# quenotl/PARESIS

Measured on AMD Instinct MI355X. Metric: Mpixels/s, 4096^2 Fresnel+refraction step, higher is better.
Workload: dtype f32; 1 GPU; 4096x4096 fp32 study grid, 1 membrane position per GPU per step, 4 propagation distances z={1.6,3.6,5.2,7.2} m: 4 x (Fresnel propagation + refraction) from the 2-material membrane thickness maps (transmission evaluated inside the step); 52 keV, dSM/dMO/dOD=140/1.6/3.6 m; fresnel_engine=lds, streams=1, parallelism=single GPU

## Files before the change

### paresis_amd/csrc/fresnel_p2.hip

```cpp
#include "fresnel_p2.hpp"

#include <atomic>

#include "fresnel_p2_dev.hpp"

using namespace psx;
using namespace psx::lines;
using namespace psx::p2dev;

namespace {

constexpr int TE = 512;
constexpr int TLD = 256;
constexpr int TT = TE + TLD;
constexpr int TOT2 = 16384;
constexpr int LXM = psx::p2::LXMAX;

template <int R1_, bool DUAL_>
struct G2 {
    static constexpr int R1 = R1_, M = 256 * R1, LINES = TOT2 / M, LH = DUAL_ ? LINES / 2 : LINES;
    static constexpr int MP = M + M / 32 + LXM;
    static constexpr int NBA = 32 / R1;
    static constexpr int SPL = M / 16;
    static constexpr int LB = R1 == 32 ? 5 : (R1 == 16 ? 4 : (R1 == 8 ? 3 : 2));
    static constexpr int LDP = LB | 1, LDB = 17;
    static constexpr int TPL = TLD / LINES, NCH = TPL >= 2 * LXM ? TPL / LXM : 1, CL = LXM / NCH;
    static constexpr int O_TP = LINES * MP, O_TB = O_TP + 256 * LDP, O_SA = O_TB + 16 * LDB, O_C = O_SA + LH * LXM,
                         O_UQ = O_C + NCH * LINES * LXM, O_HT = O_UQ + 2;
    static constexpr size_t lds_bytes(int ntap) { return sizeof(float2) * (size_t)(O_HT + ntap * LXM); }
    static constexpr int max_taps = (160 * 1024 / (int)sizeof(float2) - O_HT) / LXM < MAX_LINE ? (160 * 1024 / (int)sizeof(float2) - O_HT) / LXM : MAX_LINE;
    static_assert(LINES >= 2 && NBA >= 1 && max_taps >= 16, "LDS budget");
};

#define PSX_STAMP(k) PSX_STAMP_IF(k, tid == 0)

template <int R1, bool CONTIG, bool DUAL, bool QUEUE>
__global__ __launch_bounds__(TT) void k_fresnel_p2(LineArgs a) {
    using GE = G2<R1, DUAL>;
    constexpr int M = GE::M, LINES = GE::LINES, LH = GE::LH, MP = GE::MP, NBA = GE::NBA, SPL = GE::SPL, LDP = GE::LDP, LDB = GE::LDB;
    constexpr int NCH = GE::NCH, CL = GE::CL, TPL = GE::TPL;
    constexpr int LPG = LH;
    constexpr int LL = LH;
    static_assert(!DUAL || CONTIG, "DUAL is pass 1");
    extern __shared__ __attribute__((aligned(16))) float2 lds[];
    v2f *const Lb = reinterpret_cast<v2f *>(lds);
    v2f *const tP = Lb + GE::O_TP, *const tB = Lb + GE::O_TB;
    v2f *const SA = Lb + GE::O_SA;
    v2f *const CF = Lb + GE::O_C;
    v2f *const HT = Lb + GE::O_HT;
    int *const uq = reinterpret_cast<int *>(Lb + GE::O_UQ);
    const int tid = threadIdx.x;
    const int N = a.N, mg = a.margin;
    const int Lx = a.L - M;
    const bool upper_half = ((a.P - 1) >> 8) >= R1 / 2;

    const int ngroups = (a.nlines + LPG - 1) / LPG;
    const int nwork = a.dist_inner ? ngroups : ngroups * a.n_dist;
    const int xcd = blockIdx.x & 7, slot = blockIdx.x >> 3, nslot = gridDim.x >> 3;
    const int cq = nwork >> 3, cr = nwork & 7;
    const int cstart = xcd * cq + (xcd < cr ? xcd : cr), clen = cq + (xcd < cr ? 1 : 0);
    const int nunits = slot < clen ? (clen - slot + nslot - 1) / nslot : 0;
    const int nsub = DUAL ? (a.n_dist + 1) / 2 : a.n_dist;
    const int nj = a.dist_inner ? nunits * nsub : nunits;
    constexpr bool DYN = QUEUE;
    const int nsubr = a.dist_inner ? nsub : 1;
    auto item = [&](int j, int &d, int &g) __attribute__((always_inline)) {
        if (a.dist_inner) {
            const int u = j / nsub;
            d = j - u * nsub;
            g = cstart + (DYN ? uq[u & 3] : slot + u * nslot);
        } else {
            const int wk = cstart + (DYN ? uq[j & 3] : slot + j * nslot);
            d = wk / ngroups;
            g = wk - d * ngroups;
        }
    };
    auto valid = [&](int j) __attribute__((always_inline)) { return DYN ? uq[(j / nsubr) & 3] >= 0 : j < nj; };
    auto qcount = [&](int v) __attribute__((always_inline)) { return &a.queue[16 * (xcd + 8 * v)]; };
    auto share = [&](int v) __attribute__((always_inline)) { return v < clen ? (clen - v + nslot - 1) / nslot : 0; };
    bool dry = false, own_dry = false;
    const int myshare = share(slot);
    auto steal = [&]() __attribute__((always_inline)) {
        const int ln = tid & 63;
        for (int attempt = 0; attempt < 2; ++attempt) {
            const int v = ln;
            bool avail = false;
            if (v < nslot && v != slot)
                avail = __hip_atomic_load(qcount(v), __ATOMIC_RELAXED, __HIP_MEMORY_SCOPE_AGENT) < (unsigned)share(v);
            const unsigned long long m = __ballot(avail);
            if (m == 0ull) {
                dry = true;
                return -1;
            }
            const unsigned long long hi = m >> ((slot + 1) & 63);
            const int pick = hi ? (slot + 1 + __builtin_ctzll(hi)) : __builtin_ctzll(m);
            unsigned k = 0u;
            if (ln == 0) k = atomicAdd(qcount(pick), 1u);
            k = __builtin_amdgcn_readfirstlane(k);
            if (k < (unsigned)share(pick)) return pick + (int)k * nslot;
        }
        return -1;
    };

    unsigned first2 = 0u;
    if (DYN && tid == TE) first2 = atomicAdd(qcount(slot), 2u);
    for (int idx = tid; idx < 256 * GE::LB; idx += TT) {
        const float2 wv = a.twA[idx];
        tP[(idx / GE::LB) * LDP + idx % GE::LB] = (v2f){wv.x, wv.y};
    }
    for (int idx = tid; idx < 256; idx += TT) {
        const float2 w = a.twB[idx];
        tB[(idx >> 4) * LDB + (idx & 15)] = (v2f){w.x, w.y};
    }
    {
        const int ntap = DUAL ? 2 * nsub : a.n_dist;
        for (int idx = tid; idx < ntap * LXM; idx += TT) {
            const float2 h = a.H[idx / LXM][M + idx % LXM];
            HT[idx] = (v2f){h.x, h.y};
        }
    }
    if constexpr (DYN) {
        if (tid == TE) {
            uq[0] = first2 < (unsigned)myshare ? slot + (int)first2 * nslot : -1;
            uq[1] = first2 + 1u < (unsigned)myshare ? slot + (int)(first2 + 1u) * nslot : -1;
        }
        lds_barrier();
    }

    if (tid >= TE) {
        const int lt = tid - TE;
        constexpr int STEP = TLD / LL, NLD = M / (2 * STEP), PSTEP = STEP + STEP / 32;
        static_assert(TLD % LL == 0 && NLD * STEP == M / 2, "sample ownership covers M / 2 samples of every line");
        constexpr bool AFFL = (STEP % 32 == 0);
        const int line = CONTIG ? lt / STEP : lt % LL, i0 = CONTIG ? lt % STEP : lt / LL;
        const int nmir = LL * 2 * mg;
        const int lm = lt % LL;
        int im = -1, jm = 0;
        if (lt < nmir) {
            const int r = lt / LL;
            im = r < mg ? r + 1 : N - 1 - 2 * mg + r;
            jm = r < mg ? N + 2 * mg - 1 - im : 2 * N - 3 - im;
        }
        float2 *base = lds + line * MP;
        const int ja = i0 + N + 2 * mg - 1, jb = i0 - 1;
        const int oa = phys(ja), ob = phys(jb);
        float2 *sa_line = lds + GE::O_SA + line * LXM;

        constexpr int CH = LL / 2 > 0 ? LL / 2 : 1, STEPV = TLD / CH, NLV = M / (2 * STEPV), PSTEPV = STEPV + STEPV / 32;
        static_assert(CONTIG || (LL % 2 == 0 && IB % 2 == 0 && STEPV % 32 == 0 && NLV * STEPV == M / 2), "16-byte loads of the blocked intermediate");
        const int c2 = lt % CH, i0v = lt / CH;
        float2 *base_v = lds + 2 * c2 * MP;
        const int jav = i0v + N + 2 * mg - 1, jbv = i0v - 1;
        const int oav = phys(jav), obv = phys(jbv);
        float2 *sa_v = lds + GE::O_SA + 2 * c2 * LXM;
        const int voff_v = ((((2 * c2) / IB) * N + i0v) * IB + (2 * c2) % IB) * (int)sizeof(float2);

        float2 xs[CONTIG ? NLD : 1], xm = make_float2(0.f, 0.f);
        float4 xv[CONTIG ? 1 : NLV];
        auto fetch = [&](int j) __attribute__((always_inline)) {
            int d, g;
            item(j, d, g);
            if (a.dist_inner && d != 0) return;
            const float2 *src = a.src[d];
            const int l0 = g * LPG;
            if constexpr (!CONTIG) {
                constexpr int LLB = LL > IB ? LL / IB : 1;
                const int nblk = min(LLB, (a.nlines - l0 + IB - 1) / IB);
                const __amdgpu_buffer_rsrc_t rs = __builtin_amdgcn_make_buffer_rsrc(
                    const_cast<float2 *>(src) + ((int64_t)(l0 / IB) * N) * IB + l0 % IB, 0,
                    nblk * N * IB * (int)sizeof(float2) - (l0 % IB) * (int)sizeof(float2), 0x00020000);
#pragma unroll
                for (int k = 0; k < NLV; ++k) {
                    const v4u r = __builtin_amdgcn_raw_buffer_load_b128(rs, voff_v + k * (STEPV * IB * (int)sizeof(float2)), 0, 0);
                    xv[k] = __builtin_bit_cast(float4, r);
                }
                const int64_t pixm = ((int64_t)((l0 + lm) / IB) * N + im) * IB + (l0 + lm) % IB;
                xm = src[(im >= 0 && l0 + lm < a.nlines) ? pixm : (int64_t)0];
                return;
            } else {
                const __amdgpu_buffer_rsrc_t rs = __builtin_amdgcn_make_buffer_rsrc(
                    const_cast<float2 *>(src) + (int64_t)l0 * a.in_sl, 0, min(LL, a.nlines - l0) * (int)a.in_sl * (int)sizeof(float2), 0x00020000);
                const int voff = (line * (int)a.in_sl + i0) * (int)sizeof(float2);
#pragma unroll
                for (int k = 0; k < NLD; ++k) {
                    const v2u r = __builtin_amdgcn_raw_buffer_load_b64(rs, voff + k * (STEP * (int)sizeof(float2)), 0, 0);
                    xs[k] = __builtin_bit_cast(float2, r);
                }
                const int64_t pixm = (int64_t)im + (int64_t)(l0 + lm) * a.in_sl;
                xm = src[(im >= 0 && l0 + lm < a.nlines) ? pixm : (int64_t)0];
                return;
            }
        };
        auto spread = [&](int j) __attribute__((always_inline)) {
            int d, g;
            item(j, d, g);
            const int l0 = g * LPG;
            const bool line_ok = l0 + line < a.nlines;
            for (int jz = a.L + lt; jz < M; jz += TLD) {
                const int pz = phys(jz);
#pragma unroll
                for (int ln = 0; ln < LL; ++ln) lds[ln * MP + pz] = make_float2(0.f, 0.f);
            }
            if constexpr (!CONTIG) {
                const bool ok0 = l0 + 2 * c2 < a.nlines, ok1 = l0 + 2 * c2 + 1 < a.nlines;
#pragma unroll
                for (int k = 0; k < NLV; ++k) {
                    if (i0v + STEPV * k < N) {
                        const float2 x0 = ok0 ? make_float2(xv[k].x, xv[k].y) : make_float2(0.f, 0.f);
                        const float2 x1 = ok1 ? make_float2(xv[k].z, xv[k].w) : make_float2(0.f, 0.f);
                        base_v[oav + k * PSTEPV] = x0;
                        base_v[MP + oav + k * PSTEPV] = x1;
                        if (k > 0 || jbv >= 0) {
                            base_v[obv + k * PSTEPV] = x0;
                            base_v[MP + obv + k * PSTEPV] = x1;
                        }
                        if (STEPV * k <= LXM) {
                            const int js = jbv + STEPV * k;
                            if ((unsigned)js < (unsigned)LXM) {
                                sa_v[js] = x0;
                                sa_v[LXM + js] = x1;
                            }
                        }
                    }
                }
            }
#pragma unroll
            for (int k = 0; k < (CONTIG ? NLD : 0); ++k) {
                if (i0 + STEP * k < N) {
                    const float2 x = line_ok ? xs[k] : make_float2(0.f, 0.f);
                    if (AFFL) {
                        base[oa + k * PSTEP] = x;
                        if (k > 0 || jb >= 0) base[ob + k * PSTEP] = x;
                    } else {
                        base[phys(ja + STEP * k)] = x;
                        if (k > 0 || jb >= 0) base[phys(jb + STEP * k)] = x;
                    }
                    if (STEP * k <= LXM) {
                        const int js = jb + STEP * k;
                        if ((unsigned)js < (unsigned)LXM) sa_line[js] = x;
                    }
                }
            }
            if (im >= 0) lds[lm * MP + phys(jm)] = l0 + lm < a.nlines ? xm : make_float2(0.f, 0.f);
            for (int t = lt + TLD; t < nmir; t += TLD) {
                const int ln = t % LL, r = t / LL;
                const int i2 = r < mg ? r + 1 : N - 1 - 2 * mg + r, j2 = r < mg ? N + 2 * mg - 1 - i2 : 2 * N - 3 - i2;
                float2 x2 = make_float2(0.f, 0.f);
                if (l0 + ln < a.nlines)
                    x2 = a.src[d][a.in_blocked ? ((int64_t)((l0 + ln) / IB) * N + i2) * IB + (l0 + ln) % IB
                                            : (int64_t)i2 * a.in_si + (int64_t)(l0 + ln) * a.in_sl];
                lds[ln * MP + phys(j2)] = x2;
            }
        };
        auto fixup = [&](int j) __attribute__((always_inline)) {
            if (Lx <= 0) return;
            int d, g;
            item(j, d, g);
            int lo = lt;
            asm volatile("" : "+v"(lo));
            const int lb = lo / TPL, r = lo % TPL;
            const int lbi = DUAL ? lb % LH : lb;
            const int dd = DUAL ? 2 * d + lb / LH : d;
            const v2f *ht = HT + dd * LXM;
            const v2f *sa = SA + lbi * LXM;
            const v2f *sb = Lb + lbi * MP + M + M / 32;
            const int c = NCH > 1 ? r / LXM : 0;
            for (int mp = NCH > 1 ? r % LXM : r; mp < LXM; mp += (NCH > 1 ? LXM : TPL)) {
                v2f acc = (v2f){0.f, 0.f};
#pragma unroll
                for (int tt = 0; tt < CL; ++tt) {
                    const int t = c * CL + tt;
                    const int jx = mp >= t ? mp - t : 0;
                    const v2f dl = lds_read(sb + jx) - lds_read(sa + jx);
                    const v2f term = pk_cmul(dl, lds_read(ht + t));
                    acc += mp >= t ? term : (v2f){0.f, 0.f};
                }
                CF[(c * LINES + lb) * LXM + mp] = acc;
            }
        };

        if (valid(0)) {
            fetch(0);
            spread(0);
        }
        lds_barrier();
        int ucur = 0, usub = 0;
        auto ring_ok = [&](int u) __attribute__((always_inline)) { return uq[u & 3] >= 0; };
        for (int j = 0; DYN ? ring_ok(ucur) : j < nj; ++j) {
            const bool last_sub = usub + 1 == nsubr;
            const bool more = DYN ? ring_ok(last_sub ? ucur + 1 : ucur) : j + 1 < nj;
            lds_barrier();
            if (a.stamps && lt == 0 && j == a.stamp_j) a.stamps[(size_t)blockIdx.x * 32 + 16] = wall_clock64();
            const bool qround = DYN && lt < 64 && usub == 0;
            const bool claiming = qround && ring_ok(ucur + 1);
            unsigned mine = 0xffffffffu;
            if (claiming && !own_dry && lt == 0) mine = atomicAdd(qcount(slot), 1u);
            if (more) fetch(j + 1);
            if (a.stamps && lt == 0 && j == a.stamp_j) a.stamps[(size_t)blockIdx.x * 32 + 17] = wall_clock64();
            fixup(j);
            lds_barrier();
            lds_barrier();
            if (a.stamps && lt == 0 && j == a.stamp_j) a.stamps[(size_t)blockIdx.x * 32 + 18] = wall_clock64();
            __builtin_amdgcn_s_setprio(3);
            if (more) spread(j + 1);
            __builtin_amdgcn_s_setprio(0);
            if (qround) {
                int unit = -1;
                if (claiming) {
                    const unsigned k = __builtin_amdgcn_readfirstlane(mine);
                    if (k < (unsigned)myshare) unit = slot + (int)k * nslot;
                    else own_dry = true;
                    if (unit < 0 && !dry) unit = steal();
                }
                if (lt == 0) uq[(ucur + 2) & 3] = unit;
            }
            if (last_sub) {
                usub = 0;
                ++ucur;
            } else {
                ++usub;
            }
            if (a.stamps && lt == 0 && j == a.stamp_j) a.stamps[(size_t)blockIdx.x * 32 + 19] = wall_clock64();
            lds_barrier();
            if (a.stamps && lt == 0 && j == a.stamp_j) a.stamps[(size_t)blockIdx.x * 32 + 20] = wall_clock64();
        }
        if (DYN && lt < 64) {
            unsigned prev = 0u;
            if (lt == 0) {
                __threadfence();
                prev = atomicAdd(&a.queue[16 * 256], 1u);
            }
            prev = __builtin_amdgcn_readfirstlane(prev);
            if (prev == gridDim.x - 1) {
                for (int wq = lt; wq < (int)gridDim.x; wq += 64) atomicExch(&a.queue[16 * wq], 0u);
                if (lt == 0) atomicExch(&a.queue[16 * 256], 0u);
            }
        }
        return;
    }

    const int w = tid >> 6, ln = tid & 63;
    const int n3 = ln & 15, blk = ((ln >> 4) & 1) * 2 + (ln >> 5);
    const int slabw = spectrum::slab_of_lane(ln);
    const v2f *rowB = tB + n3 * LDB;
    constexpr int RPL = R1 / 4;
    const int G0 = DUAL ? 4 * w + blk : 2 * (w / RPL) * R1 + 4 * (w % RPL) + blk, G1 = G0 + (DUAL ? 32 : R1);
    const int S0 = DUAL ? 64 * w + slabw : 2 * (w / RPL) * SPL + 64 * (w % RPL) + slabw, S1 = S0 + (DUAL ? LH * SPL : SPL);
    auto block_ptr = [&](int G) __attribute__((always_inline)) { return Lb + (G / R1) * MP + (G % R1) * BSTR + n3; };
    auto slab_ptr = [&](int S) __attribute__((always_inline)) {
        const int sl = S % SPL;
        return Lb + (S / SPL) * MP + 16 * sl + (sl >> 1);
    };
    const bool fwdA_on = !(DUAL && R1 == 32) || tid < TE / 2;
    const int sg = __builtin_amdgcn_readfirstlane(w % RPL);
    const int hlane = spectrum::unit_of_lane<8>(sg, 0, ln);
    static_assert(spectrum::unit_of_lane<8>(0, 1, 0) == 64, "stride of a lane's loads");
    constexpr int NBAF = DUAL ? (R1 == 32 ? 1 : NBA / 2) : NBA;
    if (a.stamps && tid == 0) a.stamps[(size_t)blockIdx.x * 32 + 0] = wall_clock64();
    lds_barrier();
    if (a.stamps && tid == 0) a.stamps[(size_t)blockIdx.x * 32 + 1] = wall_clock64();
    int eu = 0, es = 0;
    for (int j = 0; DYN ? uq[eu & 3] >= 0 : j < nj; ++j) {
        int d, g;
        item(j, d, g);
        const int l0 = g * LPG;
        if (++es == nsubr) {
            es = 0;
            ++eu;
        }
        PSX_STAMP(2);

        if (fwdA_on) {
            v2f v[NBAF][R1], pw[5];
#pragma unroll
            for (int i = 0; i < NBAF; ++i) {
                const int b = tid + TE * i, n = b & 255;
                const v2f *p = Lb + (b >> 8) * MP + n + (n >> 5);
#pragma unroll
                for (int q = 0; q < R1; ++q) v[i][q] = p[q * BSTR];
            }
#pragma unroll
            for (int i = 0; i < NBAF; ++i) {
                const int b = tid + TE * i;
                v2f *p = Lb + (b >> 8) * MP + (b & 255) + ((b & 255) >> 5);
                DftPk<R1, false>::run(v[i]);
                __builtin_amdgcn_sched_barrier(0);
                if (i == 0) tw_powers<R1>(pw, tP + (tid & 255) * LDP);
                twiddle_A2<R1, false>(v[i], pw);
#pragma unroll
                for (int q = 0; q < R1; ++q) p[q * BSTR] = v[i][q];
            }
        }
        float4 hh[8], hh1[DUAL ? 8 : 1];
        {
            const float4 *h4 = reinterpret_cast<const float4 *>(a.H[DUAL ? 2 * d : d]) + hlane;
#pragma unroll
            for (int q = 0; q < 8; ++q) hh[q] = h4[64 * q];
        }
        PSX_STAMP(3);
        lds_barrier();
        PSX_STAMP(4);

        {
            v2f wt[16];
#pragma unroll
            for (int q = 1; q < 16; ++q) wt[q] = lds_read(rowB + q);
            wt[0] = (v2f){1.f, 0.f};
            v2f *p0 = block_ptr(G0), *p1 = block_ptr(G1);
            v2f v0[16], v1[DUAL ? 1 : 16];
#pragma unroll
            for (int q = 0; q < 16; ++q) v0[q] = lds_read(p0 + offB(q));
            if constexpr (DUAL) {
                const float4 *h4b = reinterpret_cast<const float4 *>(a.H[2 * d + 1]) + hlane;
                __builtin_amdgcn_sched_barrier(0);
#pragma unroll
                for (int q = 0; q < 8; ++q) hh1[q] = h4b[64 * q];
                __builtin_amdgcn_sched_barrier(0);
            } else {
#pragma unroll
                for (int q = 0; q < 16; ++q) v1[q] = lds_read(p1 + offB(q));
            }
            fwdB_regs(v0, wt);
#pragma unroll
            for (int q = 0; q < 16; ++q) p0[offB(q)] = v0[q];
            if constexpr (!DUAL) {
                fwdB_regs(v1, wt);
#pragma unroll
                for (int q = 0; q < 16; ++q) p1[offB(q)] = v1[q];
            }
        }
        PSX_STAMP(5);
        wave_sync();
        PSX_STAMP(6);

        {
            v2f *b0 = slab_ptr(S0), *b1 = slab_ptr(S1);
            v2f x[16], y[16];
#pragma unroll
            for (int q = 0; q < 16; ++q) x[q] = lds_read(b0 + q);
            if constexpr (!DUAL) {
#pragma unroll
                for (int q = 0; q < 16; ++q) y[q] = lds_read(b1 + q);
            }
            DftPk<16, false>::run(x);
            if constexpr (DUAL) {
#pragma unroll
                for (int q = 0; q < 8; ++q) {
                    y[2 * q] = pk_cmul(x[2 * q], (v2f){hh[q].x, hh[q].y});
                    y[2 * q + 1] = pk_cmul(x[2 * q + 1], (v2f){hh[q].z, hh[q].w});
                }
                DftPk<16, true>::run(y);
#pragma unroll
                for (int q = 0; q < 16; ++q) b0[q] = y[q];
#pragma unroll
                for (int q = 0; q < 8; ++q) {
                    x[2 * q] = pk_cmul(x[2 * q], (v2f){hh1[q].x, hh1[q].y});
                    x[2 * q + 1] = pk_cmul(x[2 * q + 1], (v2f){hh1[q].z, hh1[q].w});
                }
                DftPk<16, true>::run(x);
#pragma unroll
                for (int q = 0; q < 16; ++q) b1[q] = x[q];
            } else {
#pragma unroll
                for (int q = 0; q < 8; ++q) {
                    x[2 * q] = pk_cmul(x[2 * q], (v2f){hh[q].x, hh[q].y});
                    x[2 * q + 1] = pk_cmul(x[2 * q + 1], (v2f){hh[q].z, hh[q].w});
                }
                DftPk<16, true>::run(x);
#pragma unroll
                for (int q = 0; q < 16; ++q) b0[q] = x[q];
                DftPk<16, false>::run(y);
#pragma unroll
                for (int q = 0; q < 8; ++q) {
                    y[2 * q] = pk_cmul(y[2 * q], (v2f){hh[q].x, hh[q].y});
                    y[2 * q + 1] = pk_cmul(y[2 * q + 1], (v2f){hh[q].z, hh[q].w});
                }
                DftPk<16, true>::run(y);
#pragma unroll
                for (int q = 0; q < 16; ++q) b1[q] = y[q];
            }
        }
        PSX_STAMP(7);
        wave_sync();
        PSX_STAMP(8);

        {
            v2f wt[16];
#pragma unroll
            for (int q = 1; q < 16; ++q) wt[q] = lds_read(rowB + q);
            wt[0] = (v2f){1.f, 0.f};
            v2f *p0 = block_ptr(G0), *p1 = block_ptr(G1);
            v2f v0[16], v1[16];
#pragma unroll
            for (int q = 0; q < 16; ++q) v0[q] = lds_read(p0 + offB(q));
#pragma unroll
            for (int q = 0; q < 16; ++q) v1[q] = lds_read(p1 + offB(q));
            invB_regs(v0, wt);
#pragma unroll
            for (int q = 0; q < 16; ++q) p0[offB(q)] = v0[q];
            invB_regs(v1, wt);
#pragma unroll
            for (int q = 0; q < 16; ++q) p1[offB(q)] = v1[q];
        }
        PSX_STAMP(9);
        lds_barrier();
        PSX_STAMP(10);

        {
            v2f v[NBA][R1], cf[NBA], pw[5];
#pragma unroll
            for (int i = 0; i < NBA; ++i) {
                const int b = tid + TE * i, n = b & 255;
                const v2f *p = Lb + (b >> 8) * MP + n + (n >> 5);
#pragma unroll
                for (int q = 0; q < R1; ++q) v[i][q] = p[q * BSTR];
                cf[i] = CF[(b >> 8) * LXM + (n & (LXM - 1))];
#pragma unroll
                for (int c = 1; c < NCH; ++c) cf[i] += CF[(c * LINES + (b >> 8)) * LXM + (n & (LXM - 1))];
            }
            lds_barrier();
            PSX_STAMP(11);
#pragma unroll
            for (int i = 0; i < NBA; ++i) {
                int bo = tid + TE * i;
                asm volatile("" : "+v"(bo));
                const int n = bo & 255, lb = bo >> 8;
                if (i == 0) tw_powers<R1>(pw, tP + n * LDP);
                twiddle_A2<R1, true>(v[i], pw);
                __builtin_amdgcn_sched_barrier(0);
                DftPk<R1, true>::run(v[i]);
                const int ifirst = n - (a.P - 1);
                const int lbu = __builtin_amdgcn_readfirstlane(lb);
                const int dd = DUAL ? 2 * d + lbu / LH : d;
                const int l = l0 + (DUAL ? lbu % LH : lbu);
                v2f *wo = reinterpret_cast<v2f *>(a.wave_out[dd]);
                float *io = a.inten_out[dd];
                const bool lok = l < a.nlines;
                const int e0 = a.out_blocked ? ((ifirst >> IBS) * a.nlines + l) * IB + (ifirst & (IB - 1)) : ifirst;
                const int estep = a.out_blocked ? (256 / IB) * a.nlines * IB : 256;
                const int64_t wbase = a.out_blocked ? 0 : (int64_t)l * a.out_ld;
                const int welems = lok ? (a.out_blocked ? ((N + IB - 1) / IB) * IB * a.nlines : N) : 0;
                if (upper_half)
                    store_legs<R1, R1 / 2>(v[i], v[i][0] + cf[i], wo, io, wbase, welems, e0, estep, (v2f){a.gph[dd].x, a.gph[dd].y},
                                           a.scale[dd], a.accumulate);
                else
                    store_legs<R1, 0>(v[i], v[i][0] + cf[i], wo, io, wbase, welems, e0, estep, (v2f){a.gph[dd].x, a.gph[dd].y},
                                      a.scale[dd], a.accumulate);
            }
        }
        PSX_STAMP(12);
        lds_barrier();
        PSX_STAMP(13);
    }
}

__global__ void k_p2_twiddles(float2 *twA, float2 *twB, int R1, int LB) {
    const int idx = blockIdx.x * blockDim.x + threadIdx.x;
    const int M = 256 * R1;
    if (idx < 256 * LB) {
        const int n = idx / LB, b = idx % LB;
        double s, c;
        sincospi(-2.0 * (double)((n << b) % M) / (double)M, &s, &c);
        twA[idx] = make_float2((float)c, (float)s);
    }
    if (idx < 256) {
        const int n = idx >> 4, k = idx & 15;
        double s, c;
        sincospi(-2.0 * (double)((n * k) % 256) / 256.0, &s, &c);
        twB[idx] = make_float2((float)c, (float)s);
    }
}

__global__ void k_p2_perm(const double2 *__restrict__ Hh, const double2 *__restrict__ hP, float2 *__restrict__ out, int R1, int P) {
    const int p = blockIdx.x * blockDim.x + threadIdx.x;
    const int M = 256 * R1;
    if (p < M) {
        const int k1 = p >> 8, k2 = (p >> 4) & 15, k3 = p & 15;
        const double2 v = Hh[k1 + R1 * k2 + 16 * R1 * k3];
        out[spectrum::point_index(p)] = make_float2((float)(v.x / M), (float)(v.y / M));
    } else if (p < M + LXM) {
        const int t = p - M;
        const double2 v = t < P ? hP[t] : make_double2(0.0, 0.0);
        out[p] = make_float2((float)(v.x / P), (float)(v.y / P));
    }
}

int line_grid_slots(int nwork, int cap) {
    int nslot = current_cu_count() / 8;
    if (nslot > (nwork + 7) / 8) nslot = (nwork + 7) / 8;
    if (cap && nslot > cap) nslot = cap;
    return nslot;
}

template <int R1, bool CONTIG, bool DUAL, bool QUEUE = false>
int launch_t(const LineArgs &la, hipStream_t st, const char *name) {
    if constexpr (!QUEUE) {
        if (la.queue) return launch_t<R1, CONTIG, DUAL, true>(la, st, name);
    }
    using GE = G2<R1, DUAL>;
    if (int rc = allow_dynamic_lds<k_fresnel_p2<R1, CONTIG, DUAL, QUEUE>>((int)GE::lds_bytes(GE::max_taps))) return rc;
    if (la.n_dist < 1 || la.n_dist > MAX_LINE || (DUAL && !la.dist_inner))
        return fail(PSX_E_STATE, "LDS engine (power-of-two lines): %d distances, dist_inner %d", la.n_dist, la.dist_inner);
    const int ntap = DUAL ? 2 * ((la.n_dist + 1) / 2) : la.n_dist;
    if (ntap > GE::max_taps) return fail(PSX_E_STATE, "LDS engine (power-of-two lines): %d distances in one launch, %d fit", ntap, GE::max_taps);
    const int nwork = ((la.nlines + GE::LH - 1) / GE::LH) * (la.dist_inner ? 1 : la.n_dist);
    const int nslot = line_grid_slots(nwork, QUEUE ? 32 : 0);
    PSX_TIMED(name, st, k_fresnel_p2<R1, CONTIG, DUAL, QUEUE><<<8 * nslot, TT, GE::lds_bytes(ntap), st>>>(la));
    const int rc = launch_check(name);
    if constexpr (QUEUE) {
        if (rc) (void)hipMemsetAsync(la.queue, 0, sizeof(unsigned) * QUEUE_WORDS, st);
    }
    return rc;
}

template <int R1>
int launch_r(bool contig, bool dual, const LineArgs &la, hipStream_t st, const char *name) {
    if (dual) return launch_t<R1, true, true>(la, st, name);
    return contig ? launch_t<R1, true, false>(la, st, name) : launch_t<R1, false, false>(la, st, name);
}

}

namespace psx {
namespace p2 {

int pick_r1(int N, int margin) {
    const int P = N + 2 * margin, L = N + P - 1;
    for (int r1 : {4, 8, 16, 32}) {
        const int M = 256 * r1;
        if (N <= M / 2 && P <= M && L - M <= LXMAX && L - M <= N - 1) return r1;
    }
    return 0;
}

static int log2_r1(int R1) { return R1 == 32 ? 5 : (R1 == 16 ? 4 : (R1 == 8 ? 3 : 2)); }
size_t twA_elems(int R1) { return (size_t)256 * log2_r1(R1); }
int max_distances(int R1) {
    switch (R1) {
        case 4: return G2<4, false>::max_taps;
        case 8: return G2<8, false>::max_taps;
        case 16: return G2<16, false>::max_taps;
    }
    return G2<32, false>::max_taps;
}
size_t twB_elems() { return 256; }
size_t spectrum_elems(int R1) { return (size_t)256 * R1 + LXMAX; }
int lines_per_round(int R1, bool dual) { return (TOT2 / (256 * R1)) / (dual ? 2 : 1); }

int build_tables(float2 *twA, float2 *twB, int R1, hipStream_t st) {
    k_p2_twiddles<<<(256 * log2_r1(R1) + 255) / 256, 256, 0, st>>>(twA, twB, R1, log2_r1(R1));
    return launch_check("k_p2_twiddles");
}

int perm_spectrum(const double2 *Hh, const double2 *hP, float2 *out, int R1, int P, hipStream_t st) {
    const int n = 256 * R1 + LXMAX;
    PSX_TIMED("k_kern_perm", st, k_p2_perm<<<(n + 255) / 256, 256, 0, st>>>(Hh, hP, out, R1, P));
    return launch_check("k_p2_perm");
}

int launch(int R1, bool contig, bool dual, const lines::LineArgs &la, hipStream_t st, const char *name) {
    switch (R1) {
        case 4: return launch_r<4>(contig, dual, la, st, name);
        case 8: return launch_r<8>(contig, dual, la, st, name);
        case 16: return launch_r<16>(contig, dual, la, st, name);
        case 32: return launch_r<32>(contig, dual, la, st, name);
    }
    return fail(PSX_E_UNSUPPORTED, "LDS engine (power-of-two lines): unsupported radix %d", R1);
}

}
}
```

### paresis_amd/csrc/fresnel_p2_dev.hpp

```cpp
#pragma once
#include "fresnel_stages.hpp"

namespace psx {
namespace p2dev {

using namespace psx::lines;

constexpr int BSTR = 256 + 8;

namespace spectrum {
__host__ __device__ constexpr int slab_of_lane(int ln) { return (ln & 32) + ((ln & 31) < 16 ? 2 * (ln & 31) : 2 * ((ln & 31) - 16) + 1); }
__host__ __device__ constexpr int lane_of_slab(int s) { return (s & 32) + ((s & 1) ? 16 : 0) + ((s & 31) >> 1); }
template <int UPS>
__host__ __device__ constexpr int unit_of_lane(int g, int q, int ln) { return (g * UPS + q) * 64 + ln; }
template <int UPS>
__host__ __device__ constexpr int unit_of_slab(int s, int q) { return unit_of_lane<UPS>(s >> 6, q, lane_of_slab(s & 63)); }
__host__ __device__ constexpr int point_index(int p) { return 2 * unit_of_slab<8>(p >> 4, (p & 15) >> 1) + (p & 1); }
__host__ __device__ constexpr int pair_index(int p) { return unit_of_slab<16>(p >> 4, p & 15); }

constexpr bool lanes_invert() {
    for (int ln = 0; ln < 64; ++ln)
        if (lane_of_slab(slab_of_lane(ln)) != ln || slab_of_lane(lane_of_slab(ln)) != ln) return false;
    return true;
}
template <typename F>
constexpr bool is_bijection(F f, int m) {
    bool seen[8192] = {};
    for (int p = 0; p < m; ++p) {
        const int i = f(p);
        if (i < 0 || i >= m || seen[i]) return false;
        seen[i] = true;
    }
    return true;
}
constexpr bool reader_meets_builder(int m) {
    for (int g = 0; g < m / 1024; ++g)
        for (int q = 0; q < 8; ++q)
            for (int ln = 0; ln < 64; ++ln) {
                const int p = 16 * (64 * g + slab_of_lane(ln)) + 2 * q;
                if (point_index(p) != 2 * unit_of_lane<8>(g, q, ln) || point_index(p + 1) != 2 * unit_of_lane<8>(g, q, ln) + 1) return false;
                if (q == 0 && (pair_index(p) != unit_of_lane<16>(g, 0, ln) || pair_index(p + 15) != unit_of_lane<16>(g, 15, ln))) return false;
            }
    return true;
}
static_assert(lanes_invert(), "slab_of_lane and lane_of_slab are inverse permutations of the 64 lanes");
static_assert(is_bijection(point_index, 256 * 4) && is_bijection(point_index, 256 * 8) && is_bijection(point_index, 256 * 16) &&
                  is_bijection(point_index, 256 * 32) && is_bijection(pair_index, 256 * 32),
              "the table order is a bijection of the M positions for R1 = 4, 8, 16, 32");
static_assert(reader_meets_builder(256 * 4) && reader_meets_builder(256 * 32), "a lane's loads find its own slab");
}

template <int R, bool CONJ>
__device__ __forceinline__ v2f tw_apply(v2f x, v2f w) {
    return CONJ ? pk_cmulc(x, w) : pk_cmul(x, w);
}
template <int R>
__device__ __forceinline__ void tw_powers(v2f (&pw)[5], const v2f *row) {
    pw[0] = lds_read(row);
    if constexpr (R >= 4) pw[1] = lds_read(row + 1);
    if constexpr (R >= 8) pw[2] = lds_read(row + 2);
    if constexpr (R >= 16) pw[3] = lds_read(row + 3);
    if constexpr (R == 32) pw[4] = lds_read(row + 4);
}
template <int R, bool CONJ>
__device__ __forceinline__ void twiddle_A2(v2f (&v)[R], const v2f (&pw)[5]) {
    constexpr int H = R >= 16 ? 16 : R;
    v2f t[H];
    t[1] = pw[0];
    if constexpr (R >= 4) t[2] = pw[1];
    if constexpr (R >= 8) t[4] = pw[2];
    if constexpr (R >= 16) t[8] = pw[3];
    v2f t16 = (v2f){1.f, 0.f};
    if constexpr (R == 32) t16 = pw[4];
    if constexpr (R >= 4) t[3] = pk_cmul(t[1], t[2]);
    if constexpr (R >= 8) {
#pragma unroll
        for (int r = 1; r < 4; ++r) t[4 + r] = pk_cmul(t[4], t[r]);
    }
    if constexpr (R >= 16) {
#pragma unroll
        for (int r = 1; r < 8; ++r) t[8 + r] = pk_cmul(t[8], t[r]);
    }
#pragma unroll
    for (int q = 1; q < H; ++q) v[q] = tw_apply<R, CONJ>(v[q], t[q]);
    if constexpr (R == 32) {
#pragma unroll
        for (int q = 16; q < 32; ++q) v[q] = tw_apply<R, CONJ>(v[q], t16);
#pragma unroll
        for (int q = 17; q < 32; ++q) v[q] = tw_apply<R, CONJ>(v[q], t[q - 16]);
    }
}

__device__ __forceinline__ int offB(int q) { return 16 * q + (q >> 1); }

__device__ __forceinline__ void fwdB_regs(v2f (&v)[16], const v2f (&w)[16]) {
    DftPk<16, false>::run(v);
#pragma unroll
    for (int q = 1; q < 16; ++q) v[q] = pk_cmul(v[q], w[q]);
}
__device__ __forceinline__ void invB_regs(v2f (&v)[16], const v2f (&w)[16]) {
#pragma unroll
    for (int q = 1; q < 16; ++q) v[q] = pk_cmulc(v[q], w[q]);
    DftPk<16, true>::run(v);
}

template <int R, int Q0>
__device__ __forceinline__ void store_legs(const v2f (&v)[R], v2f vw, v2f *wo, float *io, int64_t wbase, int welems, int e0, int estep,
                                           v2f gp, float sc, int accumulate) {
    if (wo) {
        const __amdgpu_buffer_rsrc_t rs = __builtin_amdgcn_make_buffer_rsrc(wo + wbase, 0, (int)((unsigned)welems * 8u), 0x00020000);
        const bool plain = gp.x == 1.f && gp.y == 0.f;
        unsigned off = ((unsigned)e0 + (unsigned)Q0 * (unsigned)estep) * 8u;
#pragma unroll
        for (int q = Q0; q <= R; ++q) {
            const v2f x = q < R ? v[q < R ? q : 0] : vw;
            const v2f r = plain ? x : pk_cmul_s(x, gp);
            __builtin_amdgcn_raw_buffer_store_b64(__builtin_bit_cast(v2u, r), rs, (int)off, 0, 0);
            off += (unsigned)estep * 8u;
        }
    }
    if (io) {
        const __amdgpu_buffer_rsrc_t rs = __builtin_amdgcn_make_buffer_rsrc(io + wbase, 0, (int)((unsigned)welems * 4u), 0x00020000);
        unsigned off = ((unsigned)e0 + (unsigned)Q0 * (unsigned)estep) * 4u;
#pragma unroll
        for (int q = Q0; q <= R; ++q) {
            const v2f x = q < R ? v[q < R ? q : 0] : vw;
            float I = sc * (x.x * x.x + x.y * x.y);
            if (accumulate) I += __builtin_bit_cast(float, __builtin_amdgcn_raw_buffer_load_b32(rs, (int)off, 0, 0));
            __builtin_amdgcn_raw_buffer_store_b32(__builtin_bit_cast(unsigned, I), rs, (int)off, 0, 0);
            off += (unsigned)estep * 4u;
        }
    }
}

template <int CNT>
__device__ __forceinline__ void store_legs_range(const v2f (&v)[CNT], int q0, v2f *wo, float *io, int64_t wbase, int welems, int e0, int estep,
                                                 v2f gp, float sc, int accumulate) {
    if (wo) {
        const __amdgpu_buffer_rsrc_t rs = __builtin_amdgcn_make_buffer_rsrc(wo + wbase, 0, (int)((unsigned)welems * 8u), 0x00020000);
        const bool plain = gp.x == 1.f && gp.y == 0.f;
        unsigned off = ((unsigned)e0 + (unsigned)q0 * (unsigned)estep) * 8u;
#pragma unroll
        for (int q = 0; q < CNT; ++q) {
            const v2f r = plain ? v[q] : pk_cmul_s(v[q], gp);
            __builtin_amdgcn_raw_buffer_store_b64(__builtin_bit_cast(v2u, r), rs, (int)off, 0, 0);
            off += (unsigned)estep * 8u;
        }
    }
    if (io) {
        const __amdgpu_buffer_rsrc_t rs = __builtin_amdgcn_make_buffer_rsrc(io + wbase, 0, (int)((unsigned)welems * 4u), 0x00020000);
        unsigned off = ((unsigned)e0 + (unsigned)q0 * (unsigned)estep) * 4u;
#pragma unroll
        for (int q = 0; q < CNT; ++q) {
            float I = sc * (v[q].x * v[q].x + v[q].y * v[q].y);
            if (accumulate) I += __builtin_bit_cast(float, __builtin_amdgcn_raw_buffer_load_b32(rs, (int)off, 0, 0));
            __builtin_amdgcn_raw_buffer_store_b32(__builtin_bit_cast(unsigned, I), rs, (int)off, 0, 0);
            off += (unsigned)estep * 4u;
        }
    }
}

}
}
```

Before: 62420 Mpixel/s.

## Reuse forward-A transform across DUAL distance rounds via register snapshot/restore

In the DUAL pass-1 path, the loader threads snapshot the forward-A transformed lines into registers after the first distance round and restore them into LDS for the following rounds. The forward-A FFT stage and its barrier are then skipped on every round after the first, and the two distance halves swap slabs to keep the snapshot region intact. A workgroup-scoped LDS counter with a spin-wait orders the snapshot against compute-wave writes. The cost is extra register pressure on the loader waves, one more LDS word, and a busy-wait that could stall the compute waves.

```diff
diff --git a/paresis_amd/csrc/fresnel_p2.hip b/paresis_amd/csrc/fresnel_p2.hip
--- a/paresis_amd/csrc/fresnel_p2.hip
+++ b/paresis_amd/csrc/fresnel_p2.hip
@@ -26,7 +26,7 @@
     static constexpr int LDP = LB | 1, LDB = 17;
     static constexpr int TPL = TLD / LINES, NCH = TPL >= 2 * LXM ? TPL / LXM : 1, CL = LXM / NCH;
     static constexpr int O_TP = LINES * MP, O_TB = O_TP + 256 * LDP, O_SA = O_TB + 16 * LDB, O_C = O_SA + LH * LXM,
-                         O_UQ = O_C + NCH * LINES * LXM, O_HT = O_UQ + 2;
+                         O_UQ = O_C + NCH * LINES * LXM, O_HT = O_UQ + 3;
     static constexpr size_t lds_bytes(int ntap) { return sizeof(float2) * (size_t)(O_HT + ntap * LXM); }
     static constexpr int max_taps = (160 * 1024 / (int)sizeof(float2) - O_HT) / LXM < MAX_LINE ? (160 * 1024 / (int)sizeof(float2) - O_HT) / LXM : MAX_LINE;
     static_assert(LINES >= 2 && NBA >= 1 && max_taps >= 16, "LDS budget");
@@ -49,6 +49,7 @@
     v2f *const CF = Lb + GE::O_C;
     v2f *const HT = Lb + GE::O_HT;
     int *const uq = reinterpret_cast<int *>(Lb + GE::O_UQ);
+    int *const snap_flag = uq + 4;
     const int tid = threadIdx.x;
     const int N = a.N, mg = a.margin;
     const int Lx = a.L - M;
@@ -260,7 +261,7 @@
             asm volatile("" : "+v"(lo));
             const int lb = lo / TPL, r = lo % TPL;
             const int lbi = DUAL ? lb % LH : lb;
-            const int dd = DUAL ? 2 * d + lb / LH : d;
+            const int dd = DUAL ? 2 * d + 1 - lb / LH : d;
             const v2f *ht = HT + dd * LXM;
             const v2f *sa = SA + lbi * LXM;
             const v2f *sb = Lb + lbi * MP + M + M / 32;
@@ -279,6 +280,21 @@
             }
         };
 
+        constexpr int NSNAP = DUAL ? M * LH / TLD : 1;
+        static_assert(!DUAL || (M % TLD == 0 && NSNAP * TLD == M * LH && TLD % 32 == 0), "snapshot ownership covers the first half");
+        v2f snap[NSNAP];
+        v2f *const snap_base = Lb + phys(lt);
+        auto snap_off = [](int k) __attribute__((always_inline)) { return ((k * TLD) / M) * MP + phys((k * TLD) % M); };
+        auto snapshot = [&]() __attribute__((always_inline)) {
+#pragma unroll
+            for (int k = 0; k < NSNAP; ++k) snap[k] = lds_read(snap_base + snap_off(k));
+        };
+        auto restore = [&]() __attribute__((always_inline)) {
+#pragma unroll
+            for (int k = 0; k < NSNAP; ++k) snap_base[snap_off(k)] = snap[k];
+        };
+
+        if (lt == 0) uq[4] = 0;
         if (valid(0)) {
             fetch(0);
             spread(0);
@@ -289,8 +305,19 @@
         for (int j = 0; DYN ? ring_ok(ucur) : j < nj; ++j) {
             const bool last_sub = usub + 1 == nsubr;
             const bool more = DYN ? ring_ok(last_sub ? ucur + 1 : ucur) : j + 1 < nj;
-            lds_barrier();
+            const RoundPlan rp = round_plan(DUAL, usub, nsubr);
+            round_barrier(rp, RB_FWD_A);
             if (a.stamps && lt == 0 && j == a.stamp_j) a.stamps[(size_t)blockIdx.x * 32 + 16] = wall_clock64();
+            if constexpr (DUAL) {
+                if (rp.snapshot) {
+                    __builtin_amdgcn_s_setprio(3);
+                    snapshot();
+                    asm volatile("s_waitcnt lgkmcnt(0)" ::: "memory");
+                    __builtin_amdgcn_s_setprio(0);
+                    if ((lt & 63) == 0) __hip_atomic_fetch_add(snap_flag, 1, __ATOMIC_RELAXED, __HIP_MEMORY_SCOPE_WORKGROUP);
+                }
+                if (a.stamps && lt == 0 && j == a.stamp_j) a.stamps[(size_t)blockIdx.x * 32 + 24] = wall_clock64();
+            }
             const bool qround = DYN && lt < 64 && usub == 0;
             const bool claiming = qround && ring_ok(ucur + 1);
             unsigned mine = 0xffffffffu;
@@ -298,11 +325,16 @@
             if (more) fetch(j + 1);
             if (a.stamps && lt == 0 && j == a.stamp_j) a.stamps[(size_t)blockIdx.x * 32 + 17] = wall_clock64();
             fixup(j);
-            lds_barrier();
-            lds_barrier();
+            round_barrier(rp, RB_PRIVATE);
+            round_barrier(rp, RB_REGS);
             if (a.stamps && lt == 0 && j == a.stamp_j) a.stamps[(size_t)blockIdx.x * 32 + 18] = wall_clock64();
-            __builtin_amdgcn_s_setprio(3);
-            if (more) spread(j + 1);
+            if (!(DUAL && rp.restore)) __builtin_amdgcn_s_setprio(3);
+            if constexpr (DUAL) {
+                if (rp.restore) restore();
+                else if (more) spread(j + 1);
+            } else {
+                if (more) spread(j + 1);
+            }
             __builtin_amdgcn_s_setprio(0);
             if (qround) {
                 int unit = -1;
@@ -321,7 +353,7 @@
                 ++usub;
             }
             if (a.stamps && lt == 0 && j == a.stamp_j) a.stamps[(size_t)blockIdx.x * 32 + 19] = wall_clock64();
-            lds_barrier();
+            round_barrier(rp, RB_NEXT);
             if (a.stamps && lt == 0 && j == a.stamp_j) a.stamps[(size_t)blockIdx.x * 32 + 20] = wall_clock64();
         }
         if (DYN && lt < 64) {
@@ -359,18 +391,19 @@
     if (a.stamps && tid == 0) a.stamps[(size_t)blockIdx.x * 32 + 0] = wall_clock64();
     lds_barrier();
     if (a.stamps && tid == 0) a.stamps[(size_t)blockIdx.x * 32 + 1] = wall_clock64();
-    int eu = 0, es = 0;
+    int eu = 0, es = 0, snaps_taken = 0;
     for (int j = 0; DYN ? uq[eu & 3] >= 0 : j < nj; ++j) {
         int d, g;
         item(j, d, g);
         const int l0 = g * LPG;
+        const RoundPlan rp = round_plan(DUAL, es, nsubr);
         if (++es == nsubr) {
             es = 0;
             ++eu;
         }
         PSX_STAMP(2);
 
-        if (fwdA_on) {
+        if (fwdA_on && rp.forward_a) {
             v2f v[NBAF][R1], pw[5];
 #pragma unroll
             for (int i = 0; i < NBAF; ++i) {
@@ -398,7 +431,7 @@
             for (int q = 0; q < 8; ++q) hh[q] = h4[64 * q];
         }
         PSX_STAMP(3);
-        lds_barrier();
+        round_barrier(rp, RB_FWD_A);
         PSX_STAMP(4);
 
         {
@@ -422,7 +455,7 @@
             }
             fwdB_regs(v0, wt);
 #pragma unroll
-            for (int q = 0; q < 16; ++q) p0[offB(q)] = v0[q];
+            for (int q = 0; q < 16; ++q) (DUAL ? p1 : p0)[offB(q)] = v0[q];
             if constexpr (!DUAL) {
                 fwdB_regs(v1, wt);
 #pragma unroll
@@ -434,7 +467,7 @@
         PSX_STAMP(6);
 
         {
-            v2f *b0 = slab_ptr(S0), *b1 = slab_ptr(S1);
+            v2f *b0 = slab_ptr(DUAL ? S1 : S0), *b1 = slab_ptr(DUAL ? S0 : S1);
             v2f x[16], y[16];
 #pragma unroll
             for (int q = 0; q < 16; ++q) x[q] = lds_read(b0 + q);
@@ -452,6 +485,13 @@
                 DftPk<16, true>::run(y);
 #pragma unroll
                 for (int q = 0; q < 16; ++q) b0[q] = y[q];
+                if (rp.snapshot) {
+                    snaps_taken += TLD / 64;
+                    PSX_STAMP(25);
+                    while (*(const volatile __attribute__((address_space(3))) int *)snap_flag - snaps_taken < 0) __builtin_amdgcn_s_sleep(1);
+                    __builtin_amdgcn_fence(__ATOMIC_ACQUIRE, "workgroup", "local");
+                    PSX_STAMP(26);
+                }
 #pragma unroll
                 for (int q = 0; q < 8; ++q) {
                     x[2 * q] = pk_cmul(x[2 * q], (v2f){hh1[q].x, hh1[q].y});
@@ -503,7 +543,7 @@
             for (int q = 0; q < 16; ++q) p1[offB(q)] = v1[q];
         }
         PSX_STAMP(9);
-        lds_barrier();
+        round_barrier(rp, RB_PRIVATE);
         PSX_STAMP(10);
 
         {
@@ -518,7 +558,7 @@
 #pragma unroll
                 for (int c = 1; c < NCH; ++c) cf[i] += CF[(c * LINES + (b >> 8)) * LXM + (n & (LXM - 1))];
             }
-            lds_barrier();
+            round_barrier(rp, RB_REGS);
             PSX_STAMP(11);
 #pragma unroll
             for (int i = 0; i < NBA; ++i) {
@@ -531,7 +571,7 @@
                 DftPk<R1, true>::run(v[i]);
                 const int ifirst = n - (a.P - 1);
                 const int lbu = __builtin_amdgcn_readfirstlane(lb);
-                const int dd = DUAL ? 2 * d + lbu / LH : d;
+                const int dd = DUAL ? 2 * d + 1 - lbu / LH : d;
                 const int l = l0 + (DUAL ? lbu % LH : lbu);
                 v2f *wo = reinterpret_cast<v2f *>(a.wave_out[dd]);
                 float *io = a.inten_out[dd];
@@ -549,7 +589,7 @@
             }
         }
         PSX_STAMP(12);
-        lds_barrier();
+        round_barrier(rp, RB_NEXT);
         PSX_STAMP(13);
     }
 }
diff --git a/paresis_amd/csrc/fresnel_p2_dev.hpp b/paresis_amd/csrc/fresnel_p2_dev.hpp
--- a/paresis_amd/csrc/fresnel_p2_dev.hpp
+++ b/paresis_amd/csrc/fresnel_p2_dev.hpp
@@ -49,6 +49,35 @@
               "the table order is a bijection of the M positions for R1 = 4, 8, 16, 32");
 static_assert(reader_meets_builder(256 * 4) && reader_meets_builder(256 * 32), "a lane's loads find its own slab");
 }
+
+enum RoundBarrier { RB_FWD_A = 0, RB_PRIVATE, RB_REGS, RB_NEXT, RB_COUNT };
+struct RoundPlan {
+    bool forward_a, snapshot, restore;
+    constexpr bool has(RoundBarrier b) const { return b == RB_FWD_A ? forward_a : true; }
+};
+__host__ __device__ constexpr RoundPlan round_plan(bool dual, int sub, int nsub) {
+    return RoundPlan{!dual || sub == 0, dual && sub == 0 && nsub > 1, dual && sub + 1 < nsub};
+}
+__device__ __forceinline__ void round_barrier(const RoundPlan &rp, RoundBarrier b) {
+    if (rp.has(b)) lds_barrier();
+}
+constexpr bool rounds_consistent() {
+    for (int nsub = 1; nsub <= 16; ++nsub) {
+        bool held = false;
+        for (int s = 0; s < nsub; ++s) {
+            const RoundPlan rp = round_plan(true, s, nsub), pl = round_plan(false, s, nsub);
+            if (!pl.forward_a || pl.snapshot || pl.restore) return false;
+            if (rp.forward_a != (s == 0) || (s > 0 && !held)) return false;
+            if (rp.snapshot) held = true;
+            if (rp.snapshot && !rp.forward_a) return false;
+            if (rp.restore && !held) return false;
+            if (s > 0 && !round_plan(true, s - 1, nsub).restore) return false;
+        }
+        if (round_plan(true, nsub - 1, nsub).restore || held != (nsub > 1)) return false;
+    }
+    return true;
+}
+static_assert(rounds_consistent(), "the rounds of a DUAL line group");
 
 template <int R, bool CONJ>
 __device__ __forceinline__ v2f tw_apply(v2f x, v2f w) {
```

Result: faster. 63390 Mpixel/s (median of 6 runs) (+1.5%).
